# 2892931976/consensus-rs

Measured on AMD Instinct MI355X. Metric: BFT instance-rounds/sec (whole node), N=64 f=21, 1/2/4/8 GPUs; bit-exact, higher is better.
Workload: dtype u64

## Files before the change

### consensus-rs_amd/csrc/bft_common.h

```cpp
#pragma once
#include <stdint.h>

#if defined(__HIPCC__)
#include <hip/hip_runtime.h>
#define BFT_FN __host__ __device__ inline
#else
#define BFT_FN inline
#endif

namespace bft {

struct Params {
    uint32_t n;
    uint32_t seg;
    uint32_t heights;
    uint32_t hcap;
    uint32_t max_ticks;
    uint32_t block_period;
    uint64_t genesis_time;
    uint64_t seed;
    uint32_t thr16;
    uint32_t byz_count;
    uint32_t crash_thr32;
    uint32_t crash_on;
// ... 563 lines not shown
constexpr uint32_t SFX_DWORDS = 64, SFX_BODY_DW = 60, SFX_LEN_DW = 63, SFX_DEV_LEN_DW = 60, SFX_DEV_DW = 61;
constexpr uint32_t SFX_PAD = 18, SFX_BUF = 112, PFX_WORDS = 9;
BFT_FN uint32_t header_suffix(uint64_t* wb, const uint8_t* addr20, uint64_t seed, uint32_t inst, uint32_t h,
                              uint32_t prop, uint32_t var, uint64_t time) {
    HdrWriter w(wb);
    header_suffix_fields(w, addr20, seed, inst, h, prop, var, time);
    const uint32_t len = 8u * w.wi + w.fill;
    wb[w.wi++] = w.acc | (0x01ull << (8u * w.fill));
    while (w.wi < SFX_DWORDS / 2u - 1u) wb[w.wi++] = 0;
    wb[SFX_DWORDS / 2u - 1u] = (uint64_t)len << 32;
    return len;
}
BFT_FN uint32_t header_suffix_strided(uint32_t* sb, uint32_t stride, const uint8_t* addr20, uint64_t seed,
                                      uint32_t inst, uint32_t h, uint32_t prop, uint32_t var, uint64_t time) {
    HdrWriter w(sb, stride);
    header_suffix_fields(w, addr20, seed, inst, h, prop, var, time);
    const uint32_t len = 8u * w.wi + w.fill;
    w.store(w.wi++, w.acc | (0x01ull << (8u * w.fill)));
    while (w.wi < SFX_BODY_DW / 2u) w.store(w.wi++, 0);
    sb[(uint64_t)SFX_DEV_LEN_DW * stride] = len;
    return len;
}
BFT_FN uint32_t header_prefix(uint64_t* wb, const uint32_t prev[8]) {
    HdrWriter w(wb);
    header_prefix_fields(w, prev);
    const uint32_t len = 8u * w.wi + w.fill;
    wb[w.wi++] = w.acc;
    while (w.wi < PFX_WORDS) wb[w.wi++] = 0;
    return len;
}
struct PfxSel { uint32_t lo, hi; };
BFT_FN constexpr PfxSel pfx_sel(uint32_t idx) {
    uint32_t out[8] = {12, 12, 12, 12, 12, 12, 12, 12};
    uint32_t pos = 0;
    for (uint32_t i = 0; i < 4; ++i) {
        if ((idx >> i) & 1u) out[pos++] = 4;
        out[pos++] = i;
    }
    return PfxSel{out[0] | out[1] << 8 | out[2] << 16 | out[3] << 24, out[4] | out[5] << 8 | out[6] << 16 | out[7] << 24};
}
BFT_FN uint32_t perm_bytes(uint32_t s0, uint32_t s1, uint32_t sel) {
#if defined(__HIP_DEVICE_COMPILE__)
    return __builtin_amdgcn_perm(s0, s1, sel);
#else
    const uint64_t v = ((uint64_t)s0 << 32) | s1;
    uint32_t d = 0;
    for (int k = 0; k < 4; ++k) {
        const uint32_t q = (sel >> (8 * k)) & 0xffu;
        d |= (q < 8 ? (uint32_t)((v >> (8 * q)) & 0xffu) : 0u) << (8 * k);
    }
    return d;
#endif
}
BFT_FN uint32_t header_prefix_perm(uint64_t* wb, const uint32_t prev[8], const PfxSel* tbl) {
    uint64_t acc = 0x2000dc9dull;
    uint32_t fill = 4, wi = 0;
#pragma unroll
    for (int i = 0; i < 8; ++i) {
        const uint32_t w = prev[i];
        const uint32_t idx = ((((w >> 7) & 0x01010101u) * 0x10204080u) >> 28);
        const PfxSel sel = tbl[idx];
        const uint64_t v = (uint64_t)perm_bytes(0xccccccccu, w, sel.lo) | ((uint64_t)perm_bytes(0xccccccccu, w, sel.hi) << 32);
        const uint32_t n = 4u + (uint32_t)__builtin_popcount(idx);
        const uint32_t sh = 8u * fill, nf = fill + n;
        const uint64_t lo = acc | (v << sh);
        wb[wi] = lo;
        const bool full = nf >= 8u;
        acc = full ? (sh ? v >> (64u - sh) : 0ull) : lo;
        wi += full ? 1u : 0u;
        fill = full ? nf - 8u : nf;
    }
    wb[wi] = acc;
#pragma unroll
    for (uint32_t k = 1; k <= 4; ++k) wb[wi + k] = 0;
    return 8u * wi + fill;
}
BFT_FN uint32_t align_bytes(uint32_t hi, uint32_t lo, uint32_t r) {
#if defined(__HIP_DEVICE_COMPILE__)
    return __builtin_amdgcn_alignbyte(hi, lo, r);
#else
    return (uint32_t)((((uint64_t)hi << 32) | lo) >> (8u * r));
#endif
}
BFT_FN uint32_t splice_blocks(uint32_t len_p, uint32_t len_s) { return (len_p + len_s + 136u) / 136u; }
BFT_FN uint32_t splice_word(const uint32_t* sx, uint32_t r, const uint32_t* pw, uint32_t w, uint32_t nb) {
    uint32_t v = align_bytes(sx[w + 1u], sx[w], r);
    if (w < 2u * PFX_WORDS) v |= pw[w];
    if (w == 34u * nb - 1u) v ^= 0x80000000u;
    return v;
}
BFT_FN uint32_t header_words(uint64_t* wb, const uint32_t prev[8], const uint8_t* addr20, uint64_t seed,
                             uint32_t inst, uint32_t h, uint32_t prop, uint32_t var, uint64_t time) {
    HdrWriter w(wb);
    header_fields(w, prev, addr20, seed, inst, h, prop, var, time);
    return w.finish();
}
BFT_FN uint32_t header_raw(uint64_t* wb, const uint32_t prev[8], const uint8_t* addr20, uint64_t seed,
                           uint32_t inst, uint32_t h, uint32_t prop, uint32_t var, uint64_t time) {
    HdrWriter w(wb);
    header_fields(w, prev, addr20, seed, inst, h, prop, var, time);
    const uint32_t len = 8u * w.wi + w.fill;
    if (w.fill) wb[w.wi] = w.acc;
    return len;
}

BFT_FN void lane_block_hash(uint8_t* buf, const uint32_t prev[8], const uint8_t* addr20, uint64_t seed,
                            uint32_t inst, uint32_t h, uint32_t prop, uint32_t var, uint64_t time,
                            uint32_t out[8]) {
    uint64_t* wb = (uint64_t*)buf;
    const uint32_t nb = header_words(wb, prev, addr20, seed, inst, h, prop, var, time);
    uint64_t a[25];
#pragma unroll
    for (int i = 0; i < 25; ++i) a[i] = 0;
#pragma unroll 1
    for (uint32_t blk = 0; blk < nb; ++blk) {
        const uint64_t* w = wb + 17u * blk;
#pragma unroll
        for (int i = 0; i < 17; ++i) a[i] ^= w[i];
        keccak_f1600(a);
    }
#pragma unroll
    for (int i = 0; i < 4; ++i) { out[2 * i] = (uint32_t)a[i]; out[2 * i + 1] = (uint32_t)(a[i] >> 32); }
}

BFT_FN uint32_t header_prefix_regs(const uint32_t prev[8], const PfxSel* tbl, uint32_t pw[2 * PFX_WORDS]) {
    uint64_t wv[PFX_WORDS];
#pragma unroll
    for (uint32_t k = 0; k < PFX_WORDS; ++k) wv[k] = 0;
    uint64_t acc = 0x2000dc9dull;
    uint32_t fill = 4, wi = 0;
#pragma unroll
    for (uint32_t i = 0; i < 8; ++i) {
        const uint32_t w = prev[i];
        const uint32_t idx = ((((w >> 7) & 0x01010101u) * 0x10204080u) >> 28);
        const PfxSel sel = tbl[idx];
        const uint64_t v = (uint64_t)perm_bytes(0xccccccccu, w, sel.lo) | ((uint64_t)perm_bytes(0xccccccccu, w, sel.hi) << 32);
        const uint32_t n = 4u + (uint32_t)__builtin_popcount(idx);
        const uint32_t sh = 8u * fill, nf = fill + n;
        const uint64_t lo = acc | (v << sh);
#pragma unroll
        for (uint32_t k = (1u + i) / 2u; k <= i; ++k) wv[k] = wi == k ? lo : wv[k];
        const bool full = nf >= 8u;
        acc = full ? (sh ? v >> (64u - sh) : 0ull) : lo;
        wi += full ? 1u : 0u;
        fill = full ? nf - 8u : nf;
    }
#pragma unroll
    for (uint32_t k = 4; k < PFX_WORDS; ++k) wv[k] = wi == k ? acc : wv[k];
#pragma unroll
    for (uint32_t k = 0; k < PFX_WORDS; ++k) { pw[2 * k] = (uint32_t)wv[k]; pw[2 * k + 1] = (uint32_t)(wv[k] >> 32); }
    return 8u * wi + fill;
}

#if !defined(__HIP_DEVICE_COMPILE__)
inline void spliced_block_hash(const uint32_t* sfx, const uint32_t prev[8], uint32_t out[8]) {
    for (int i = 0; i < 8; ++i) out[i] = 0;
    uint32_t buf[SFX_BUF] = {};
    for (uint32_t i = 0; i < SFX_BODY_DW; ++i) buf[SFX_PAD + i] = sfx[i];
    uint64_t pfx[PFX_WORDS + 4], ref[PFX_WORDS];
    PfxSel tbl[16];
    for (uint32_t i = 0; i < 16; ++i) tbl[i] = pfx_sel(i);
    const uint32_t lp = header_prefix_perm(pfx, prev, tbl);
    if (header_prefix(ref, prev) != lp) return;
    for (uint32_t i = 0; i < PFX_WORDS; ++i) if (ref[i] != pfx[i]) return;
    uint32_t pr[2 * PFX_WORDS];
    if (header_prefix_regs(prev, tbl, pr) != lp) return;
    for (uint32_t i = 0; i < PFX_WORDS; ++i) if (pr[2 * i] != (uint32_t)ref[i] || pr[2 * i + 1] != (uint32_t)(ref[i] >> 32)) return;
    uint32_t pw[2 * PFX_WORDS];
    for (uint32_t i = 0; i < PFX_WORDS; ++i) { pw[2 * i] = (uint32_t)pfx[i]; pw[2 * i + 1] = (uint32_t)(pfx[i] >> 32); }
    const uint32_t c = 72u - lp, nb = splice_blocks(lp, sfx[SFX_LEN_DW]);
    const uint32_t* sx = buf + (c >> 2);
    uint64_t a[25] = {};
    for (uint32_t blk = 0; blk < nb; ++blk) {
        for (uint32_t i = 0; i < 17; ++i) {
            const uint32_t w = 34u * blk + 2u * i;
            a[i] ^= (uint64_t)splice_word(sx, c & 3u, pw, w, nb) | ((uint64_t)splice_word(sx, c & 3u, pw, w + 1u, nb) << 32);
        }
        keccak_f1600(a);
    }
    for (int i = 0; i < 4; ++i) { out[2 * i] = (uint32_t)a[i]; out[2 * i + 1] = (uint32_t)(a[i] >> 32); }
}
#endif

template <uint32_t STRIDE = 1>
BFT_FN uint64_t byz_mask64(uint64_t seed, uint32_t inst, uint32_t f, uint8_t* perm) {
    auto at = [&](uint32_t i) -> uint8_t& { return perm[(i >> 2) * 4u * STRIDE + (i & 3u)]; };
    for (uint32_t i = 0; i < 64u; ++i) at(i) = (uint8_t)i;
    uint64_t mask = 0;
    if (f > 64u) f = 64u;
    for (uint32_t i = 0; i < f; ++i) {
        uint32_t w[4];
        philox(seed, inst, i, 0, DOM_BYZ, w);
        const uint32_t j = i + w[0] % (64u - i);
        const uint8_t t = at(i); at(i) = at(j); at(j) = t;
        mask |= 1ull << at(i);
    }
    return mask;
}
constexpr uint32_t SPEC_VALID = 0x80000000u;
BFT_FN bool spec_block64(uint64_t seed, uint32_t inst, uint32_t x, uint64_t byz, uint32_t tip_w0, uint32_t& j,
                         uint32_t& var) {
    j = tip_w0 & 63u;
    uint64_t v1m = 0;
    if ((byz >> j) & 1ull) {
        uint32_t w[4];
        philox(seed, inst, x, 0, DOM_SPLIT, w);
        v1m = ((uint64_t)w[0] | ((uint64_t)w[1] << 32)) & ~(1ull << j);
    }
    const uint64_t hon = ~byz;
    const bool k0 = __builtin_popcountll(byz | (hon & ~v1m)) > 42, k1 = __builtin_popcountll(byz | (hon & v1m)) > 42;
    var = k1 ? 1u : 0u;
    return k0 != k1;
}
BFT_FN uint32_t spec_word(uint32_t j, uint32_t var, uint32_t seed_next) { return SPEC_VALID | j | (var << 8) | (seed_next << 16); }

BFT_FN uint32_t seed_from_hash(const uint8_t* h, uint32_t n, bool le = false) {
    if (le) {
        uint64_t v = 0;
        for (int i = 7; i >= 0; --i) v = (v << 8) | h[i];
        return (uint32_t)(v % n);
    }
    uint64_t be = 0;
    for (int i = 0; i < 8; ++i) be = (be << 8) | h[i];
    uint64_t a = be % n;
    uint64_t t = (0xffffffffffffffffull % n + 1ull) % n;
    return (uint32_t)((a * t) % n);
}
BFT_FN uint32_t seed_from_words(uint32_t w0, uint32_t w1, uint32_t n, bool le) {
    uint8_t hb[8];
    for (int q = 0; q < 4; ++q) { hb[q] = (uint8_t)(w0 >> (8 * q)); hb[4 + q] = (uint8_t)(w1 >> (8 * q)); }
    return seed_from_hash(hb, n, le);
}

}
```

### consensus-rs_amd/csrc/kern_fast.hip

```cpp
#include "bft_hip.h"
#include "bft_fast64.h"

namespace bft {

#ifndef BFT_FAST_WAVES_PER_SIMD
#define BFT_FAST_WAVES_PER_SIMD 4
#endif
#ifndef BFT_FAST_LOSSLESS_WAVES_PER_SIMD
#define BFT_FAST_LOSSLESS_WAVES_PER_SIMD 4
#endif
#ifndef BFT_FAST_SEEDED_WAVES_PER_SIMD
#define BFT_FAST_SEEDED_WAVES_PER_SIMD 4
#endif
template <bool LOSSY, bool SEEDED>
__global__ __launch_bounds__(64, SEEDED ? BFT_FAST_SEEDED_WAVES_PER_SIMD
                                        : LOSSY ? BFT_FAST_WAVES_PER_SIMD : BFT_FAST_LOSSLESS_WAVES_PER_SIMD)
void bft_consensus_fast_kernel(Params p) {
    extern __shared__ uint8_t lds[];
#ifndef BFT_CONSENSUS_PRIO
#define BFT_CONSENSUS_PRIO 2
#endif
    __builtin_amdgcn_s_setprio(BFT_CONSENSUS_PRIO);
    Fast64<WaveHip, LOSSY, SEEDED> sim(p, lds, blockIdx.x);
    sim.run();
// ... 103 lines not shown
__device__ inline void pair_header_hash(const uint32_t* sb, const uint32_t* pw, uint32_t odd, uint32_t len_p,
                                        uint32_t len_s, uint32_t prev[8], uint32_t* dst) {
    const uint32_t c = 72u - len_p, r = c & 3u, nb = splice_blocks(len_p, len_s);
    const uint32_t* sx = sb + (c >> 2) + odd;
    uint32_t X[25];
#pragma unroll
    for (int i = 0; i < 25; ++i) X[i] = 0;
#pragma unroll
    for (uint32_t i = 0; i < 17; ++i) {
        uint32_t v = align_bytes(sx[2u * i + 1u], sx[2u * i], r);
        if (i < PFX_WORDS) v |= pw[2u * i];
        X[i] ^= v;
    }
    if (odd & (nb == 1u)) X[16] ^= 0x80000000u;
    keccak_f1600_pair(X, odd);
#pragma unroll 1
    for (uint32_t blk = 1; blk < nb; ++blk) {
        const uint32_t k0 = (c >> 2) + odd + 34u * blk;
#pragma unroll
        for (uint32_t i = 0; i < 17; ++i) {
            uint32_t ka = k0 + 2u * i, kb = ka + 1u;
            if (BFT_CHAIN_COMPACT) { ka = ka < CHAIN_SB_ZERO ? ka : CHAIN_SB_ZERO; kb = kb < CHAIN_SB_ZERO ? kb : CHAIN_SB_ZERO; }
            X[i] ^= align_bytes(sb[kb], sb[ka], r);
        }
        if (odd & (blk + 1u == nb)) X[16] ^= 0x80000000u;
        keccak_f1600_pair(X, odd);
    }
#pragma unroll
    for (int i = 0; i < 4; ++i) {
        const uint32_t o = pair_swap(X[i]);
        dst[2 * i + odd] = X[i];
        prev[2 * i] = odd ? o : X[i];
        prev[2 * i + 1] = odd ? X[i] : o;
    }
}
#endif

__constant__ PfxSel PFX_TBL[16] = {pfx_sel(0), pfx_sel(1), pfx_sel(2), pfx_sel(3), pfx_sel(4), pfx_sel(5),
                                   pfx_sel(6), pfx_sel(7), pfx_sel(8), pfx_sel(9), pfx_sel(10), pfx_sel(11),
                                   pfx_sel(12), pfx_sel(13), pfx_sel(14), pfx_sel(15)};

constexpr uint32_t CHAIN_PAIR_BLOCK = 64;
__device__ inline void set_prio(uint32_t k) {
    if (k == 1u) __builtin_amdgcn_s_setprio(1);
    else if (k == 2u) __builtin_amdgcn_s_setprio(2);
    else if (k >= 3u) __builtin_amdgcn_s_setprio(3);
}
__global__ __launch_bounds__(CHAIN_PAIR_BLOCK) void bft_hash_chain_kernel(Params p, ChainSets cs) {
    static_assert(CHAIN_PAIR_BLOCK == 64, "bft_hash_chain_kernel's barriers assume one-wave blocks");
#if defined(__HIP_DEVICE_COMPILE__)
    set_prio(p.chain_prio);
    {
        const uint32_t bps = (p.n_instances + 31u) / 32u, k = blockIdx.x / bps;
        p.sfx = const_cast<uint32_t*>(cs.sfx[k]);
        p.committed_height = const_cast<uint32_t*>(cs.ch[k]);
        p.hash = cs.hash[k];
    }
    const uint32_t blk = blockIdx.x % ((p.n_instances + 31u) / 32u);
    __shared__ __attribute__((aligned(16))) uint32_t sbuf[32 * CHAIN_SB];
    __shared__ __attribute__((aligned(16))) uint64_t pbuf[CHAIN_PB_SLOTS * (PFX_WORDS + 4)];
    __shared__ PfxSel ptbl[16];
    if (threadIdx.x < 16) ptbl[threadIdx.x] = PFX_TBL[threadIdx.x];
    __syncthreads();
    const uint32_t odd = threadIdx.x & 1u, pair = threadIdx.x >> 1;
    const uint32_t il = blk * 32u + pair;
    if (il >= p.n_instances) return;
    const uint32_t K = p.sfx_rows, x0 = p.sfx_x0;
    uint32_t x1 = x0 + K - 1u, xs = x0;
    if (p.chain_mode != CHAIN_PREDICTED) {
        const uint32_t ch = p.committed_height[il];
        x1 = ch < x1 ? ch : x1;
        if (p.chain_mode == CHAIN_REPAIR) {
            const uint32_t b = cs.bad[blockIdx.x / ((p.n_instances + 31u) / 32u)][il];
            xs = b > x0 ? b : x0;
        }
    }
    if (x1 < xs) return;
    uint32_t* sb = sbuf + pair * CHAIN_SB;
    for (uint32_t i = odd; i < SFX_PAD; i += 2u) sb[i] = 0;
    for (uint32_t i = SFX_PAD + SFX_BODY_DW + odd; i < CHAIN_SB; i += 2u) sb[i] = 0;
    const uint8_t* ph = xs == 1u ? p.genesis_hash : p.hash + ((uint64_t)il * p.rows + xs - 1u) * 32;
    uint32_t prev[8];
    for (int i = 0; i < 8; ++i)
        prev[i] = (uint32_t)ph[4 * i] | ((uint32_t)ph[4 * i + 1] << 8) | ((uint32_t)ph[4 * i + 2] << 16) |
                  ((uint32_t)ph[4 * i + 3] << 24);
    constexpr uint32_t HALF = SFX_BODY_DW / 2u;
    const uint32_t n = p.n_instances;
    const uint64_t rstride = (uint64_t)SFX_DEV_DW * n;
    const uint32_t* srow = p.sfx + il + (uint64_t)odd * HALF * n;
    uint32_t s[HALF], slen;
    {
        const uint64_t ro = (uint64_t)(xs - x0) * rstride;
#pragma unroll
        for (uint32_t i = 0; i < HALF; ++i) s[i] = srow[ro + (uint64_t)i * n];
        slen = p.sfx[il + ro + (uint64_t)SFX_DEV_LEN_DW * n];
    }
    uint64_t* pb = pbuf + (BFT_CHAIN_COMPACT ? pair : threadIdx.x) * (PFX_WORDS + 4);
    const uint32_t* pw = (const uint32_t*)pb + odd;
    for (uint32_t x = xs; x <= x1; ++x) {
        const uint32_t len_s = slen;
        if (len_s == 0u) break;
#pragma unroll
        for (uint32_t i = 0; i < HALF; ++i) sb[SFX_PAD + odd * HALF + i] = s[i];
        if (x < x1) {
            const uint64_t ro = (uint64_t)(x + 1u - x0) * rstride;
#pragma unroll
            for (uint32_t i = 0; i < HALF; ++i) s[i] = srow[ro + (uint64_t)i * n];
            slen = p.sfx[il + ro + (uint64_t)SFX_DEV_LEN_DW * n];
        }
        const uint32_t len_p = header_prefix_perm(pb, prev, ptbl);
        __syncthreads();
        pair_header_hash(sb, pw, odd, len_p, len_s, prev, (uint32_t*)(p.hash + ((uint64_t)il * p.rows + x) * 32));
        __syncthreads();
    }
#endif
}

#if defined(__HIP_DEVICE_COMPILE__)
#ifndef BFT_LANE_UNROLL
#define BFT_LANE_UNROLL 24
#endif
__device__ inline void keccak_f1600_lane(uint32_t L[25], uint32_t H[25]) {
#pragma unroll BFT_LANE_UNROLL
    for (int rnd = 0; rnd < 24; ++rnd) {
        uint32_t cl[5], ch[5], rl[5], rh[5], bl[25], bh[25];
#pragma unroll
        for (int x = 0; x < 5; ++x) {
            cl[x] = xor3_32(xor3_32(L[x], L[x + 5], L[x + 10]), L[x + 15], L[x + 20]);
            ch[x] = xor3_32(xor3_32(H[x], H[x + 5], H[x + 10]), H[x + 15], H[x + 20]);
        }
#pragma unroll
        for (int x = 0; x < 5; ++x) rotl_halves<1>(cl[(x + 1) % 5], ch[(x + 1) % 5], rl[x], rh[x]);
#define BFT_RHO_L(i, n, j) rotl_halves<n>(xor3_32(L[i], cl[((i) % 5 + 4) % 5], rl[(i) % 5]), \
                                          xor3_32(H[i], ch[((i) % 5 + 4) % 5], rh[(i) % 5]), bl[j], bh[j]);
        BFT_RHO_L(0, 0, 0) BFT_RHO_L(1, 1, 10) BFT_RHO_L(2, 62, 20) BFT_RHO_L(3, 28, 5) BFT_RHO_L(4, 27, 15)
        BFT_RHO_L(5, 36, 16) BFT_RHO_L(6, 44, 1) BFT_RHO_L(7, 6, 11) BFT_RHO_L(8, 55, 21) BFT_RHO_L(9, 20, 6)
        BFT_RHO_L(10, 3, 7) BFT_RHO_L(11, 10, 17) BFT_RHO_L(12, 43, 2) BFT_RHO_L(13, 25, 12) BFT_RHO_L(14, 39, 22)
        BFT_RHO_L(15, 41, 23) BFT_RHO_L(16, 45, 8) BFT_RHO_L(17, 15, 18) BFT_RHO_L(18, 21, 3) BFT_RHO_L(19, 8, 13)
        BFT_RHO_L(20, 18, 14) BFT_RHO_L(21, 2, 24) BFT_RHO_L(22, 61, 9) BFT_RHO_L(23, 56, 19) BFT_RHO_L(24, 14, 4)
#undef BFT_RHO_L
#pragma unroll
        for (int y = 0; y < 5; ++y)
#pragma unroll
            for (int x = 0; x < 5; ++x) {
                L[5 * y + x] = bl[5 * y + x] ^ (~bl[5 * y + (x + 1) % 5] & bl[5 * y + (x + 2) % 5]);
                H[5 * y + x] = bh[5 * y + x] ^ (~bh[5 * y + (x + 1) % 5] & bh[5 * y + (x + 2) % 5]);
            }
        L[0] ^= KECCAK_RC_LO[rnd];
        H[0] ^= KECCAK_RC_HI[rnd];
    }
}
#endif

constexpr uint32_t SFX_LDS_DW = 56;
static_assert(SFX_LDS_DW * 4u >= 213u && SFX_LDS_DW <= SFX_BODY_DW && SFX_LDS_DW % 2u == 0u, "inline suffix column");
#if defined(__HIP_DEVICE_COMPILE__)
template <bool INLINE>
__device__ inline void lane_chain(const Params& p, const ChainSets& cs, uint32_t k, uint32_t il, const PfxSel* ptbl,
                                  uint32_t* sl) {
    const uint32_t n = p.n_instances;
    const uint32_t K = p.sfx_rows, x0 = p.sfx_x0;
    uint32_t x1 = x0 + K - 1u, xs = x0;
    if (p.chain_mode != CHAIN_PREDICTED) {
        const uint32_t ch = cs.ch[k][il];
        x1 = ch < x1 ? ch : x1;
        if (p.chain_mode == CHAIN_REPAIR) {
            const uint32_t b = cs.bad[k][il];
            xs = b > x0 ? b : x0;
        }
    }
    if (x1 < xs) return;
    uint8_t* const hash = cs.hash[k];
    const uint32_t* ph = (const uint32_t*)(xs == 1u ? p.genesis_hash : hash + ((uint64_t)il * p.rows + xs - 1u) * 32);
    uint32_t prev[8];
#pragma unroll
    for (int i = 0; i < 8; ++i) prev[i] = ph[i];
    const char* const sbase = (const char*)cs.sfx[k];
    const uint32_t n4 = 4u * n;
    const uint32_t* const rec = cs.rec[k] + (uint64_t)il * p.rows * 4u;
    const bool predicted = INLINE && p.chain_mode == CHAIN_PREDICTED;
    uint64_t byz = 0;
    if (predicted) {
        byz = byz_mask64<64>(p.seed, cs.first[k] + il, p.byz_count, (uint8_t*)sl);
        cs.bad[k][il] = 0xffffffffu;
    }
    uint32_t* const pred = predicted ? cs.pred[k] + (uint64_t)il * p.heights : nullptr;
    for (uint32_t x = xs; x <= x1; ++x) {
        const uint32_t rowoff = 4u * il + (x - x0) * SFX_DEV_DW * n4;
        uint32_t len_s;
        if constexpr (INLINE) {
            uint32_t prop, var, tick;
            if (p.chain_mode == CHAIN_PREDICTED) {
                const bool ok = spec_block64(p.seed, cs.first[k] + il, x, byz, 0u, prop, var);
                pred[x - 1u] = ok ? SPEC_VALID | prop | (var << 16) : 0u;
                if (!ok) break;
                tick = x - 1u;
            } else {
                const uint4 row = *(const uint4*)(rec + 4u * x);
                prop = row.y & 0xffffu;
                var = (row.y >> 16) & 1u;
                tick = row.z;
            }
            HdrWriter w(sl, 64u);
            header_suffix_fields(w, p.addresses + 20u * prop, p.seed, cs.first[k] + il, x, prop, var,
                                 p.genesis_time + (uint64_t)p.block_period * ((uint64_t)tick + 1ull));
            len_s = 8u * w.wi + w.fill;
            w.store(w.wi++, w.acc | (0x01ull << (8u * w.fill)));
            while (w.wi < SFX_LDS_DW / 2u) w.store(w.wi++, 0);
        } else {
            len_s = *(const uint32_t*)(sbase + rowoff + SFX_DEV_LEN_DW * n4);
        }
        if (len_s == 0u) break;
        uint32_t pw[2 * PFX_WORDS];
        const uint32_t len_p = header_prefix_regs(prev, ptbl, pw);
        const uint32_t c = 72u - len_p, r = c & 3u, nb = splice_blocks(len_p, len_s);
        const int j0 = (int)(c >> 2) - (int)SFX_PAD;
        auto G = [&](uint32_t jj) -> uint32_t {
            if constexpr (INLINE) return sl[64u * jj];
            else return *(const uint32_t*)(sbase + rowoff + __umul24(jj, n4));
        };
        constexpr int BODY = INLINE ? (int)SFX_LDS_DW : (int)SFX_BODY_DW;
        auto S = [&](int j) -> uint32_t {
            const uint32_t v = G((uint32_t)(j < 0 ? 0 : j > BODY - 1 ? BODY - 1 : j));
            return ((j >= 0) & (j < BODY)) ? v : 0u;
        };
        uint32_t L[25], H[25];
#pragma unroll
        for (int i = 0; i < 25; ++i) {
            L[i] = i < (int)PFX_WORDS ? pw[2 * i] : 0u;
            H[i] = i < (int)PFX_WORDS ? pw[2 * i + 1] : 0u;
        }
        for (uint32_t blk = 0; blk < nb; ++blk) {
            uint32_t d[35];
            if (blk == 0u) {
#pragma unroll
                for (int i = 0; i < 17; ++i) d[i] = S(j0 + i);
                if constexpr (INLINE) {
#pragma unroll
                    for (int i = 17; i < 35; ++i) d[i] = G((uint32_t)(j0 + i));
                } else {
                    uint32_t vo = rowoff + __umul24((uint32_t)(j0 + 17), n4);
#pragma unroll
                    for (int i = 17; i < 35; ++i, vo += n4) d[i] = *(const uint32_t*)(sbase + vo);
                }
#pragma unroll
                for (int i = 0; i < 34; ++i) d[i] = align_bytes(d[i + 1], d[i], r);
            } else {
#pragma unroll
                for (int i = 0; i < 35; ++i) d[i] = S(j0 + 34 * (int)blk + i);
#pragma unroll
                for (int i = 0; i < 34; ++i) d[i] = align_bytes(d[i + 1], d[i], r);
            }
#pragma unroll
            for (int i = 0; i < 17; ++i) { L[i] ^= d[2 * i]; H[i] ^= d[2 * i + 1]; }
            if (blk + 1u == nb) H[16] ^= 0x80000000u;
            keccak_f1600_lane(L, H);
        }
        uint32_t* dst = (uint32_t*)(hash + ((uint64_t)il * p.rows + x) * 32);
#pragma unroll
        for (int i = 0; i < 4; ++i) { prev[2 * i] = L[i]; prev[2 * i + 1] = H[i]; }
        *(uint4*)dst = make_uint4(prev[0], prev[1], prev[2], prev[3]);
        *(uint4*)(dst + 4) = make_uint4(prev[4], prev[5], prev[6], prev[7]);
    }
}
#endif
#ifndef BFT_LANE_WAVES_PER_SIMD
#define BFT_LANE_WAVES_PER_SIMD 4
#endif

template <bool INLINE>
__global__ __launch_bounds__(64, INLINE ? BFT_LANE_WAVES_PER_SIMD : 3) void bft_hash_chain_lane_kernel(Params p, ChainSets cs) {
#if defined(__HIP_DEVICE_COMPILE__)
    set_prio(p.chain_prio);
    __shared__ PfxSel ptbl[16];
    extern __shared__ uint32_t sfx_lds[];
    if (threadIdx.x < 16) ptbl[threadIdx.x] = PFX_TBL[threadIdx.x];
    __syncthreads();
    const uint32_t bps = (p.n_instances + 63u) / 64u, tasks = cs.count * bps;
    for (uint32_t t = blockIdx.x; t < tasks; t += gridDim.x) {
        const uint32_t k = t / bps, il = (t % bps) * 64u + threadIdx.x;
        if (il < p.n_instances)
            lane_chain<INLINE>(p, cs, k, il, ptbl, INLINE ? sfx_lds + threadIdx.x : nullptr);
    }
#endif
}
static hipError_t launch_lane(uint32_t tasks, const ChainSets& cs, hipStream_t s, const Params& p) {
    const uint32_t g = p.chain_grid && p.chain_grid < tasks ? p.chain_grid : tasks;
    if (p.chain_inline)
        hipLaunchKernelGGL(bft_hash_chain_lane_kernel<true>, dim3(g), dim3(64), (size_t)SFX_LDS_DW * 64u * 4u, s, p, cs);
    else hipLaunchKernelGGL(bft_hash_chain_lane_kernel<false>, dim3(g), dim3(64), 0, s, p, cs);
    return hipGetLastError();
}

__global__ __launch_bounds__(256) void bft_spec_byz_kernel(Params p, ChainSets cs) {
    set_prio(p.chain_prio);
    __shared__ uint8_t perm[256 * 64];
    const uint32_t n = p.n_instances, bpl = (n + 255u) / 256u, k = blockIdx.x / bpl;
    const uint32_t il = (blockIdx.x % bpl) * 256u + threadIdx.x;
    if (il >= n) return;
    cs.byz[k][il] = byz_mask64(p.seed, cs.first[k] + il, p.byz_count, perm + 64u * threadIdx.x);
    cs.bad[k][il] = 0xffffffffu;
}
__device__ inline uint64_t spec_time(const Params& p, uint32_t tick) {
    return p.genesis_time + (uint64_t)p.block_period * ((uint64_t)tick + 1ull);
}
__global__ __launch_bounds__(256) void bft_spec_suffix_kernel(Params p, ChainSets cs) {
    set_prio(p.chain_prio);
    const uint32_t n = p.n_instances, H = p.heights;
    const uint32_t bpl = (uint32_t)(((uint64_t)n * H + 255u) / 256u), k = blockIdx.x / bpl;
    const uint32_t t = (blockIdx.x % bpl) * 256u + threadIdx.x;
    const uint32_t j = t / n, il = t - j * n;
    if (j >= H) return;
    const uint32_t x = j + 1u, inst = cs.first[k] + il;
    uint32_t* row = const_cast<uint32_t*>(cs.sfx[k]) + (uint64_t)j * SFX_DEV_DW * n + il;
    uint32_t prop, var;
    if (!spec_block64(p.seed, inst, x, cs.byz[k][il], 0u, prop, var)) {
        row[(uint64_t)SFX_DEV_LEN_DW * n] = 0u;
        cs.pred[k][(uint64_t)il * H + j] = 0u;
        return;
    }
    cs.pred[k][(uint64_t)il * H + j] = SPEC_VALID | prop | (var << 16);
    header_suffix_strided(row, n, p.addresses + 20u * prop, p.seed, inst, x, prop, var, spec_time(p, x - 1u));
}
__global__ __launch_bounds__(256) void bft_spec_verify_kernel(Params p, ChainSets cs) {
    const uint32_t n = p.n_instances, H = p.heights;
    const uint32_t bpl = (uint32_t)(((uint64_t)n * H + 255u) / 256u), k = blockIdx.x / bpl;
    const uint32_t t = (blockIdx.x % bpl) * 256u + threadIdx.x;
    const uint32_t il = t / H, x = t - il * H + 1u;
    if (il >= n) return;
    if (x > cs.ch[k][il]) return;
    const uint4 row = *(const uint4*)(cs.rec[k] + ((uint64_t)il * p.rows + x) * 4);
    const uint32_t pw = cs.pred[k][(uint64_t)il * H + x - 1u], inst = cs.first[k] + il;
    if (((pw & SPEC_VALID) != 0u) & ((row.y & 0x1ffffu) == (pw & 0x1ffffu)) & (row.z + 1u == x)) return;
    const uint32_t rp = row.y & 0xffffu, rv = (row.y >> 16) & 1u;
    header_suffix_strided(const_cast<uint32_t*>(cs.sfx[k]) + (uint64_t)(x - 1u) * SFX_DEV_DW * n + il, n,
                          p.addresses + 20u * rp, p.seed, inst, x, rp, rv, spec_time(p, row.z));
    atomicMin(&cs.bad[k][il], x);
}
hipError_t launch_spec_suffix(uint32_t n, const ChainSets& cs, hipStream_t s, const Params& p) {
    if (cs.count < 1 || cs.count > CHAIN_MAX_SETS || p.n_instances != n) return hipErrorInvalidValue;
    hipLaunchKernelGGL(bft_spec_byz_kernel, dim3(cs.count * ((n + 255u) / 256u)), dim3(256), 0, s, p, cs);
    const uint32_t bpl = (uint32_t)(((uint64_t)n * p.heights + 255u) / 256u);
    hipLaunchKernelGGL(bft_spec_suffix_kernel, dim3(cs.count * bpl), dim3(256), 0, s, p, cs);
    return hipGetLastError();
}
hipError_t launch_spec_verify(uint32_t n, const ChainSets& cs, hipStream_t s, const Params& p) {
    if (cs.count < 1 || cs.count > CHAIN_MAX_SETS || p.n_instances != n) return hipErrorInvalidValue;
    const uint32_t bpl = (uint32_t)(((uint64_t)n * p.heights + 255u) / 256u);
    hipLaunchKernelGGL(bft_spec_verify_kernel, dim3(cs.count * bpl), dim3(256), 0, s, p, cs);
    return hipGetLastError();
}

__global__ __launch_bounds__(CHAIN_PAIR_BLOCK) void bft_seed_chain_kernel(Params p) {
#if defined(__HIP_DEVICE_COMPILE__)
    __shared__ __attribute__((aligned(16))) uint32_t sbuf[32 * CHAIN_SB];
    __shared__ __attribute__((aligned(16))) uint64_t pbuf[CHAIN_PB_SLOTS * (PFX_WORDS + 4)];
    __shared__ PfxSel ptbl[16];
    __shared__ uint32_t slen[32];
    if (threadIdx.x < 16) ptbl[threadIdx.x] = PFX_TBL[threadIdx.x];
    __syncthreads();
    const uint32_t odd = threadIdx.x & 1u, pair = threadIdx.x >> 1;
    const uint32_t il = blockIdx.x * 32u + pair;
    if (il >= p.n_instances) return;
    const uint32_t n = p.n_instances, inst = p.first_instance + il;
    uint32_t* sb = sbuf + pair * CHAIN_SB;
    const uint64_t byz = byz_mask64(p.seed, inst, p.byz_count, (uint8_t*)(sb + SFX_PAD) + 64u * odd);
    __syncthreads();
    for (uint32_t i = odd; i < SFX_PAD; i += 2u) sb[i] = 0;
    for (uint32_t i = SFX_PAD + SFX_BODY_DW + odd; i < CHAIN_SB; i += 2u) sb[i] = 0;
    const uint8_t* ph = p.genesis_hash;
    uint32_t prev[8];
    for (int i = 0; i < 8; ++i)
        prev[i] = (uint32_t)ph[4 * i] | ((uint32_t)ph[4 * i + 1] << 8) | ((uint32_t)ph[4 * i + 2] << 16) |
                  ((uint32_t)ph[4 * i + 3] << 24);
    uint64_t* pb = pbuf + (BFT_CHAIN_COMPACT ? pair : threadIdx.x) * (PFX_WORDS + 4);
    const uint32_t* pw = (const uint32_t*)pb + odd;
    for (uint32_t x = 1; x <= p.heights; ++x) {
        uint32_t j, var;
        if (!spec_block64(p.seed, inst, x, byz, prev[0], j, var)) {
            if (!odd) p.spec[(uint64_t)x * n + il] = 0u;
            break;
        }
        if (!odd) {
            HdrWriter w(sb + SFX_PAD, 1u);
            header_suffix_fields(w, p.addresses + 20u * j, p.seed, inst, x, j, var,
                                 p.genesis_time + (uint64_t)p.block_period * (uint64_t)x);
            slen[pair] = 8u * w.wi + w.fill;
            w.store(w.wi++, w.acc | (0x01ull << (8u * w.fill)));
            while (w.wi < SFX_BODY_DW / 2u) w.store(w.wi++, 0);
        }
        const uint32_t len_p = header_prefix_perm(pb, prev, ptbl);
        __syncthreads();
        pair_header_hash(sb, pw, odd, len_p, slen[pair], prev, (uint32_t*)(p.hash + ((uint64_t)il * p.rows + x) * 32));
        if (!odd) p.spec[(uint64_t)x * n + il] = spec_word(j, var, seed_from_words(prev[0], prev[1], 64u, true));
        __syncthreads();
    }
#endif
}
hipError_t launch_seed_chain(uint32_t n, hipStream_t s, const Params& p) {
    hipLaunchKernelGGL(bft_seed_chain_kernel, dim3((n + 31u) / 32u), dim3(CHAIN_PAIR_BLOCK), 0, s, p);
    return hipGetLastError();
}

__global__ __launch_bounds__(64) void bft_hash_chain_wave_kernel(Params p, ChainSets cs) {
    __shared__ __attribute__((aligned(16))) uint32_t sb[SFX_BUF];
    __shared__ __attribute__((aligned(16))) uint32_t pf[KW_PFX_DW];
    set_prio(p.chain_prio);
    const uint32_t lane = threadIdx.x;
    const uint32_t bps = 8u * ((p.n_instances + 7u) / 8u), k = blockIdx.x / bps, b = blockIdx.x % bps;
    p.sfx = const_cast<uint32_t*>(cs.sfx[k]);
    p.committed_height = const_cast<uint32_t*>(cs.ch[k]);
    p.hash = cs.hash[k];
    const uint32_t per = bps >> 3;
    const uint32_t il = (b & 7u) * per + (b >> 3);
    if (il >= p.n_instances) return;
    const uint32_t K = p.sfx_rows, x0 = p.sfx_x0;
    const uint32_t ch = p.committed_height[il];
    const uint32_t x1 = ch < x0 + K - 1u ? ch : x0 + K - 1u;
    if (x1 < x0) return;
    const uint32_t* ph = (const uint32_t*)(x0 == 1u ? p.genesis_hash : p.hash + ((uint64_t)il * p.rows + x0 - 1u) * 32);
    const uint32_t a_prev = lane < 8u ? ph[lane] : 0u;
    WaveHip wv;
    kw50_chain(wv, lane, sb, pf, p.sfx + il, (uint64_t)SFX_DEV_DW * p.n_instances, p.n_instances, a_prev,
               x1 - x0 + 1u, (uint32_t*)(p.hash + ((uint64_t)il * p.rows + x0) * 32));
}

hipError_t launch_hash_suffix(uint32_t n, uint32_t x0, uint32_t rows, uint32_t* sfx, bool loop, hipStream_t s,
                              Params p) {
    p.sfx = sfx;
    p.sfx_rows = rows;
    p.sfx_x0 = x0;
    if (loop) hipLaunchKernelGGL(bft_hash_suffix_loop_kernel, dim3((n + 255u) / 256u), dim3(256), 0, s, p);
    else hipLaunchKernelGGL(bft_hash_suffix_kernel, dim3((uint32_t)(((uint64_t)n * rows + 255u) / 256u)), dim3(256), 0, s, p);
    return hipGetLastError();
}
// ... 29 lines not shown
```

Baseline: 3.519 billion.

## Cache suffix header per proposer and write only changed tail words in LDS column

The inline hash-chain path used to rebuild the whole per-row block-suffix column in LDS every height. It now keeps the proposer/address head and only rewrites it when the proposer changes. Only the tail is re-encoded, using a specialized writer with precomputed msgpack encoding, and just the words past the previous high-water mark get zeroed. It also adds opaque-register tricks and assumes so the compiler keeps lane indexing and addressing cheap. The added state tracking and assumptions add complexity and could break bit-exactness if any invariant is wrong.

```diff
diff --git a/consensus-rs_amd/csrc/bft_common.h b/consensus-rs_amd/csrc/bft_common.h
--- a/consensus-rs_amd/csrc/bft_common.h
+++ b/consensus-rs_amd/csrc/bft_common.h
@@ -739,6 +739,183 @@
     return 8u * wi + fill;
 }
 
+#if defined(BFT_CHECK_ASSUME)
+#define BFT_ASSUME(x) do { if (!(x)) __builtin_trap(); } while (0)
+#elif defined(__clang__)
+#define BFT_ASSUME(x) __builtin_assume(x)
+#else
+#define BFT_ASSUME(x) do { if (!(x)) __builtin_unreachable(); } while (0)
+#endif
+constexpr uint32_t SFX_LDS_DW = 56, SFX_COL_WORDS = SFX_LDS_DW / 2u;
+constexpr uint32_t SFX_MAX_LEN = 212;
+static_assert(SFX_LDS_DW * 4u >= SFX_MAX_LEN + 1u && SFX_LDS_DW <= SFX_BODY_DW && SFX_LDS_DW % 2u == 0u, "inline suffix column");
+constexpr uint32_t SFX_HEAD_WORDS = 10, SFX_HEAD_FILL = 2;
+constexpr uint64_t SFX_HEAD_ACC = 0x2000ull;
+static_assert(44u + 35u + 3u == 8u * SFX_HEAD_WORDS + SFX_HEAD_FILL, "the head ends two bytes into word 10");
+static_assert((0x2000dcull >> (8u * (3u - SFX_HEAD_FILL))) == SFX_HEAD_ACC, "those bytes are the header's last two");
+BFT_FN bool suffix_head_strided(uint32_t* sb, uint32_t stride, const uint8_t* addr20) {
+    HdrWriter w(sb, stride);
+    w.put_address(addr20);
+    w.put(0x2000dcull, 3);
+    for (int i = 0; i < 4; ++i) w.put(0, 8);
+    w.put(0x2000dcull, 3);
+    return w.wi == SFX_HEAD_WORDS && w.fill == SFX_HEAD_FILL && w.acc == SFX_HEAD_ACC;
+}
+template <uint32_t STRIDE>
+struct SfxTail {
+    uint32_t* sb;
+    uint64_t acc;
+    uint32_t fill, wi;
+    BFT_FN explicit SfxTail(uint32_t* s) : sb(s), acc(SFX_HEAD_ACC), fill(SFX_HEAD_FILL), wi(SFX_HEAD_WORDS) {}
+    BFT_FN void store(uint32_t i, uint64_t v) {
+        BFT_ASSUME(i < SFX_COL_WORDS);
+        sb[2u * i * STRIDE] = (uint32_t)v;
+        sb[(2u * i + 1u) * STRIDE] = (uint32_t)(v >> 32);
+    }
+    BFT_FN void put(uint64_t v, uint32_t n) {
+        const uint32_t sh = 8u * fill, nf = fill + n;
+        const uint64_t lo = acc | (v << sh);
+        store(wi, lo);
+        const bool full = nf >= 8u;
+        acc = full ? (v >> 1) >> (63u - sh) : lo;
+        wi += full ? 1u : 0u;
+        fill = nf & 7u;
+    }
+    BFT_FN void put_hash_word(uint32_t w, const PfxSel* tbl) {
+        const uint32_t idx = ((((w >> 7) & 0x01010101u) * 0x10204080u) >> 28);
+        const PfxSel sel = tbl[idx];
+        put((uint64_t)perm_bytes(0xccccccccu, w, sel.lo) | ((uint64_t)perm_bytes(0xccccccccu, w, sel.hi) << 32),
+            4u + (uint32_t)__builtin_popcount(idx));
+    }
+    BFT_FN void put_zeros32() {
+        store(wi, acc);
+        store(wi + 1u, 0);
+        store(wi + 2u, 0);
+        store(wi + 3u, 0);
+        acc = 0;
+        wi += 4u;
+    }
+};
+BFT_FN uint32_t bswap_u32(uint32_t v) { return (v >> 24) | ((v >> 8) & 0xff00u) | ((v << 8) & 0xff0000u) | (v << 24); }
+BFT_FN uint64_t msgpack_uint(uint64_t v, uint32_t& n) {
+    const uint32_t lo = (uint32_t)v, hi = (uint32_t)(v >> 32);
+    const uint64_t b5 = 0xceull | ((uint64_t)bswap_u32(lo) << 8);
+    const uint64_t b9 = 0xcfull | ((uint64_t)bswap_u32(hi) << 8) | ((uint64_t)(bswap_u32(lo) & 0xffffffu) << 40);
+    const uint32_t s3 = 0xcdu | ((lo & 0xff00u)) | ((lo & 0xffu) << 16), s2 = 0xccu | (lo << 8);
+    const uint32_t small = lo < 128u ? lo : lo < 256u ? s2 : s3;
+    n = hi ? 9u : lo < 128u ? 1u : lo < 256u ? 2u : lo < 65536u ? 3u : 5u;
+    return hi ? b9 : lo < 65536u ? (uint64_t)small : b5;
+}
+constexpr uint32_t SFX_NO_HEAD = 0x7ffffffu;
+struct SfxColumn {
+    uint32_t s;
+    BFT_FN uint32_t head_prop() const { return s >> 5; }
+    BFT_FN uint32_t hw() const { return s & 31u; }
+    BFT_FN void set_head_prop(uint32_t prop) { s = (prop << 5) | (s & 31u); }
+    BFT_FN void set_hw(uint32_t w) { s = (s & ~31u) | w; }
+};
+template <uint32_t STRIDE>
+BFT_FN uint32_t suffix_tail_words(uint32_t* sb, const PfxSel* tbl, const uint32_t tx[8], uint32_t h, uint64_t time,
+                                  SfxColumn& c) {
+    SfxTail<STRIDE> w(sb);
+#pragma unroll
+    for (int i = 0; i < 8; ++i) w.put_hash_word(tx[i], tbl);
+    w.put(0x2000dcull, 3);
+    w.put_zeros32();
+    uint32_t nh, nt;
+    const uint64_t eh = msgpack_uint(h, nh), et = msgpack_uint(time, nt);
+    w.put(eh << 16, 2u + nh);
+    w.put(et << 16, nt > 6u ? 8u : 2u + nt);
+    const bool t9 = nt > 6u;
+    w.put(t9 ? (et >> 48) | ((time & 0xffull) << 16) : 0ull, t9 ? 3u : 0u);
+    w.put(0x2065736e696f439bull, 8);
+    w.put(0xc065736162ull, 5);
+    const uint32_t len = 8u * w.wi + w.fill, wt = w.wi;
+    BFT_ASSUME(len <= SFX_MAX_LEN);
+    w.store(wt, w.acc | (0x01ull << (8u * w.fill)));
+#pragma unroll
+    for (uint32_t k = 1; k <= 4u; ++k) {
+        const uint32_t i = wt + k;
+        w.store(i < SFX_COL_WORDS ? i : SFX_COL_WORDS - 1u, 0);
+    }
+    for (uint32_t i = wt + 5u, hw = c.hw(); i <= hw; ++i) w.store(i, 0);
+    c.set_hw(wt);
+    return len;
+}
+template <uint32_t STRIDE>
+BFT_FN uint32_t suffix_tail_strided(uint32_t* sb, const PfxSel* tbl, uint64_t seed, uint32_t inst, uint32_t h,
+                                    uint32_t prop, uint32_t var, uint64_t time, SfxColumn& c) {
+    uint32_t tx[8];
+    tx_hash_words(seed, inst, h, prop, var, tx);
+    return suffix_tail_words<STRIDE>(sb, tbl, tx, h, time, c);
+}
+template <uint32_t STRIDE>
+BFT_FN SfxColumn suffix_column_start(uint32_t* sb) {
+#pragma unroll
+    for (uint32_t j = 2u * SFX_HEAD_WORDS; j < SFX_LDS_DW; ++j) sb[j * STRIDE] = 0;
+    return SfxColumn{SFX_NO_HEAD << 5};
+}
+BFT_FN void suffix_column_head(uint32_t* sb, uint32_t stride, const uint8_t* addresses, uint32_t prop, SfxColumn& c) {
+    if (prop != c.head_prop()) {
+        suffix_head_strided(sb, stride, addresses + 20u * prop);
+        c.set_head_prop(prop);
+    }
+}
+
+template <uint32_t STRIDE, bool LO, bool HI>
+BFT_FN uint32_t suffix_column_dword(const uint32_t* sb, int j) {
+    constexpr int LAST = (int)SFX_LDS_DW - 1;
+    int jc = j;
+    if (LO) jc = jc < 0 ? 0 : jc;
+    if (HI) jc = jc > LAST ? LAST : jc;
+    BFT_ASSUME(jc >= 0 && jc <= LAST);
+    uint32_t v = sb[(uint32_t)jc * STRIDE];
+    if (LO) v = j >= 0 ? v : 0u;
+    if (HI) v = j <= LAST ? v : 0u;
+    return v;
+}
+BFT_FN int splice_j0(uint32_t len_p) {
+    BFT_ASSUME(len_p >= 36u && len_p <= 68u);
+    return (int)((72u - len_p) >> 2) - (int)SFX_PAD;
+}
+template <uint32_t STRIDE>
+BFT_FN void splice_absorb(const uint32_t* sb, uint32_t len_p, uint32_t blk, uint32_t L[25], uint32_t H[25]) {
+    const int j0 = splice_j0(len_p);
+    const uint32_t r = (72u - len_p) & 3u;
+    BFT_ASSUME(j0 >= -17 && j0 <= -9 && blk <= 2u);
+    uint32_t d[35];
+    if (blk == 0u) {
+#pragma unroll
+        for (int i = 9; i < 17; ++i) d[i] = suffix_column_dword<STRIDE, true, false>(sb, j0 + i);
+#pragma unroll
+        for (int i = 17; i < 35; ++i) d[i] = suffix_column_dword<STRIDE, false, false>(sb, j0 + i);
+#pragma unroll
+        for (int i = 9; i < 34; ++i) {
+            const uint32_t v = align_bytes(d[i + 1], d[i], r);
+            if (i & 1) H[i >> 1] ^= v; else L[i >> 1] ^= v;
+        }
+    } else if (blk == 1u) {
+#pragma unroll
+        for (int i = 0; i < 31; ++i) d[i] = suffix_column_dword<STRIDE, false, false>(sb, j0 + 34 + i);
+#pragma unroll
+        for (int i = 31; i < 35; ++i) d[i] = suffix_column_dword<STRIDE, false, true>(sb, j0 + 34 + i);
+#pragma unroll
+        for (int i = 0; i < 34; ++i) {
+            const uint32_t v = align_bytes(d[i + 1], d[i], r);
+            if (i & 1) H[i >> 1] ^= v; else L[i >> 1] ^= v;
+        }
+    } else {
+#pragma unroll
+        for (int i = 0; i < 5; ++i) d[i] = suffix_column_dword<STRIDE, false, true>(sb, j0 + 68 + i);
+        d[5] = 0;
+#pragma unroll
+        for (int i = 0; i < 5; ++i) {
+            const uint32_t v = align_bytes(d[i + 1], d[i], r);
+            if (i & 1) H[i >> 1] ^= v; else L[i >> 1] ^= v;
+        }
+    }
+}
+
 #if !defined(__HIP_DEVICE_COMPILE__)
 inline void spliced_block_hash(const uint32_t* sfx, const uint32_t prev[8], uint32_t out[8]) {
     for (int i = 0; i < 8; ++i) out[i] = 0;
diff --git a/consensus-rs_amd/csrc/kern_fast.hip b/consensus-rs_amd/csrc/kern_fast.hip
--- a/consensus-rs_amd/csrc/kern_fast.hip
+++ b/consensus-rs_amd/csrc/kern_fast.hip
@@ -279,12 +279,11 @@
 }
 #endif
 
-constexpr uint32_t SFX_LDS_DW = 56;
-static_assert(SFX_LDS_DW * 4u >= 213u && SFX_LDS_DW <= SFX_BODY_DW && SFX_LDS_DW % 2u == 0u, "inline suffix column");
 #if defined(__HIP_DEVICE_COMPILE__)
 template <bool INLINE>
 __device__ inline void lane_chain(const Params& p, const ChainSets& cs, uint32_t k, uint32_t il, const PfxSel* ptbl,
-                                  uint32_t* sl) {
+                                  uint32_t* const cols) {
+    uint32_t* sl = INLINE ? cols + (il & 63u) : nullptr;
     const uint32_t n = p.n_instances;
     const uint32_t K = p.sfx_rows, x0 = p.sfx_x0;
     uint32_t x1 = x0 + K - 1u, xs = x0;
@@ -304,36 +303,45 @@
     for (int i = 0; i < 8; ++i) prev[i] = ph[i];
     const char* const sbase = (const char*)cs.sfx[k];
     const uint32_t n4 = 4u * n;
-    const uint32_t* const rec = cs.rec[k] + (uint64_t)il * p.rows * 4u;
-    const bool predicted = INLINE && p.chain_mode == CHAIN_PREDICTED;
+    auto is_predicted = [&]() -> bool {
+        uint32_t cm = p.chain_mode;
+        BFT_OPAQUE_SGPR(cm);
+        return INLINE && cm == CHAIN_PREDICTED;
+    };
     uint64_t byz = 0;
-    if (predicted) {
+    if (is_predicted()) {
         byz = byz_mask64<64>(p.seed, cs.first[k] + il, p.byz_count, (uint8_t*)sl);
         cs.bad[k][il] = 0xffffffffu;
     }
-    uint32_t* const pred = predicted ? cs.pred[k] + (uint64_t)il * p.heights : nullptr;
+    SfxColumn col{0u};
+    if constexpr (INLINE) {
+        col = suffix_column_start<64>(sl);
+        if (is_predicted()) suffix_column_head(sl, 64u, p.addresses, 0u, col);
+    }
     for (uint32_t x = xs; x <= x1; ++x) {
         const uint32_t rowoff = 4u * il + (x - x0) * SFX_DEV_DW * n4;
+        uint32_t ih = il;
+        if constexpr (INLINE) {
+            BFT_OPAQUE_VGPR(ih);
+            sl = cols + (ih & 63u);
+        }
         uint32_t len_s;
         if constexpr (INLINE) {
             uint32_t prop, var, tick;
             if (p.chain_mode == CHAIN_PREDICTED) {
                 const bool ok = spec_block64(p.seed, cs.first[k] + il, x, byz, 0u, prop, var);
-                pred[x - 1u] = ok ? SPEC_VALID | prop | (var << 16) : 0u;
+                cs.pred[k][(uint64_t)ih * p.heights + x - 1u] = ok ? SPEC_VALID | prop | (var << 16) : 0u;
                 if (!ok) break;
                 tick = x - 1u;
             } else {
-                const uint4 row = *(const uint4*)(rec + 4u * x);
+                const uint4 row = *(const uint4*)(cs.rec[k] + ((uint64_t)ih * p.rows + x) * 4u);
                 prop = row.y & 0xffffu;
                 var = (row.y >> 16) & 1u;
                 tick = row.z;
             }
-            HdrWriter w(sl, 64u);
-            header_suffix_fields(w, p.addresses + 20u * prop, p.seed, cs.first[k] + il, x, prop, var,
-                                 p.genesis_time + (uint64_t)p.block_period * ((uint64_t)tick + 1ull));
-            len_s = 8u * w.wi + w.fill;
-            w.store(w.wi++, w.acc | (0x01ull << (8u * w.fill)));
-            while (w.wi < SFX_LDS_DW / 2u) w.store(w.wi++, 0);
+            suffix_column_head(sl, 64u, p.addresses, prop, col);
+            len_s = suffix_tail_strided<64>(sl, ptbl, p.seed, cs.first[k] + il, x, prop, var,
+                                            p.genesis_time + (uint64_t)p.block_period * ((uint64_t)tick + 1ull), col);
         } else {
             len_s = *(const uint32_t*)(sbase + rowoff + SFX_DEV_LEN_DW * n4);
         }
@@ -383,7 +391,7 @@
             if (blk + 1u == nb) H[16] ^= 0x80000000u;
             keccak_f1600_lane(L, H);
         }
-        uint32_t* dst = (uint32_t*)(hash + ((uint64_t)il * p.rows + x) * 32);
+        uint32_t* dst = (uint32_t*)(hash + ((uint64_t)ih * p.rows + x) * 32);
 #pragma unroll
         for (int i = 0; i < 4; ++i) { prev[2 * i] = L[i]; prev[2 * i + 1] = H[i]; }
         *(uint4*)dst = make_uint4(prev[0], prev[1], prev[2], prev[3]);
@@ -405,9 +413,15 @@
     __syncthreads();
     const uint32_t bps = (p.n_instances + 63u) / 64u, tasks = cs.count * bps;
     for (uint32_t t = blockIdx.x; t < tasks; t += gridDim.x) {
-        const uint32_t k = t / bps, il = (t % bps) * 64u + threadIdx.x;
+        uint32_t lane = threadIdx.x;
+        if constexpr (INLINE) {
+            uint32_t z = 0u;
+            BFT_OPAQUE_VGPR(z);
+            lane = __builtin_amdgcn_mbcnt_hi(~0u, __builtin_amdgcn_mbcnt_lo(~0u, z));
+        }
+        const uint32_t k = t / bps, il = (t % bps) * 64u + lane;
         if (il < p.n_instances)
-            lane_chain<INLINE>(p, cs, k, il, ptbl, INLINE ? sfx_lds + threadIdx.x : nullptr);
+            lane_chain<INLINE>(p, cs, k, il, ptbl, sfx_lds);
     }
 #endif
 }
```

Result: no change. 3.513 billion (-0.2%).
